# caprilovel/ECG_Denoise

Hardware: AMD Instinct MI355X
Metric: ECG windows/sec (512-sample, bs2048) train step; inference forward in infer_*_windows_per_s (higher is better)
Workload: dtype f32; 1 GPU; RA-LENet 'full' train step, 1-lead 512-sample windows, batch 2048/GPU (fwd+mse/SNR/RMSE+bwd+Adam), N(0,1) inputs seed 2023, random-init weights; global_batch=2048, batch_per_gpu=2048, parallelism=dp1, sync_bn=True

## Files before the change

ecg_denoise_amd/csrc/ral_bwd.hip:

```cpp
#ifdef RAL_STAMP_TU_BWD
#define RAL_STAMP_HERE
#endif
#include "ral_device.hpp"
#include "ral_kernels.hpp"
#include <stdio.h>
#include <stdlib.h>
#include <type_traits>

RAL_STAMPS_DEFINE(ral_debug_stamps)

RAL_DEV void lds_add4(double* red, int c, float4 v) {
  atomicAdd(red + c, (double)v.x); atomicAdd(red + c + 1, (double)v.y); atomicAdd(red + c + 2, (double)v.z); atomicAdd(red + c + 3, (double)v.w);
}

template <int C, int NCH>
__global__ __launch_bounds__(512) void k_mlp_bwd(const float* __restrict__ dx2, const float* __restrict__ x1,
                                                 const float* __restrict__ upre, BlockP w, BlockP wt, BlockP gr,
                                                 float* __restrict__ dupre, float* __restrict__ dx1,
                                                 float* __restrict__ do_hm, float* __restrict__ a2c0, int N, int B,
                                                 int NE ) {
  extern __shared__ float4 smem4[];
  constexpr int LD = LDof<C>::v, HC = 4 * C / NCH, LDU = LDof<HC>::v, LPR = C / 4;
  float* Ds = reinterpret_cast<float*>(smem4);
  float* Gs = Ds + N * LD;
  float* Us = Gs + N * LD;
  float* A0 = Us + N * LDU;
  float* DC0 = A0 + N + 2;
  float* U0 = DC0 + N + 2;
  float* C0 = U0 + N;
  float* red = C0 + N;
  const int RPP = blockDim.x / LPR;
  const int cq = (threadIdx.x % LPR) * 4;
  const bool le = w.le != nullptr;
  float lw0 = 0.f, lw1 = 0.f, lw2 = 0.f;
  if (le) { lw0 = w.le[0]; lw1 = w.le[1]; lw2 = w.le[2]; }
  const float4 gam2 = *reinterpret_cast<const float4*>(w.ln2w + cq);
  float gle0 = 0.f, gle1 = 0.f, gle2 = 0.f;
  float4 dgam = make_float4(0.f, 0.f, 0.f, 0.f), dbet = make_float4(0.f, 0.f, 0.f, 0.f);

  RAL_STAMP_INIT();
  for (int win = blockIdx.x; win < B; win += gridDim.x) {
    const size_t wo = (size_t)win * N * C;
    RAL_STAMP_AT(15);
    copy_in(Ds, LD, dx2 + wo, C, N, C);
#pragma unroll 1
    for (int ch = 0; ch < NCH; ++ch) {
      const int j0 = ch * HC;
      copy_in(Us, LDU, upre + (size_t)win * N * 4 * C + j0, 4 * C, N, HC);
      __syncthreads();
      RAL_STAMP_AT(0);
      if (le && ch == 0) {
        for (int i = threadIdx.x; i < N + 2; i += blockDim.x) {
          const bool halo = (i == 0 || i == N + 1);
          const float u = halo ? 0.f : Us[(i - 1) * LDU];
          A0[i] = (halo || i > NE) ? 0.f : gelu_f(u);
          DC0[i] = 0.f;
          if (!halo) U0[i - 1] = u;
// ... 899 lines not shown
  const f32x2 k01 = {kv.x, kv.y}, k23 = {kv.z, kv.w}, v01 = {vv.x, vv.y}, v23 = {vv.z, vv.w};
  f32x2 dk01 = {0.f, 0.f}, dk23 = {0.f, 0.f}, dv01 = {0.f, 0.f}, dv23 = {0.f, 0.f};
  for (int qt = 0; qt < N; qt += 4) {
    float4 qr[4], dr[4];
    float2 st[4];
#pragma unroll
    for (int j = 0; j < 4; ++j) { qr[j] = Q4[qt + j]; dr[j] = D4[qt + j]; st[j] = S2[qt + j]; }
#pragma unroll
    for (int j = 0; j < 4; ++j) {
      const f32x2 qa = {qr[j].x, qr[j].y}, qb2 = {qr[j].z, qr[j].w}, da = {dr[j].x, dr[j].y}, db = {dr[j].z, dr[j].w};
      f32x2 t = k01 * qa;
      t = pk_fma(k23, qb2, t);
      f32x2 u = v01 * da;
      u = pk_fma(v23, db, u);
      float hs = t[0] + t[1], hd = u[0] + u[1];
      asm volatile("" : "+v"(hs), "+v"(hd));
      f32x2 sd = {hs, hd};
      sd += f32x2{st[j].x, st[j].y};
      const float p = __builtin_amdgcn_exp2f(sd[0]);
      const float ds = p * sd[1];
      dk01 = pk_fma(splat2(ds), qa, dk01);
      dk23 = pk_fma(splat2(ds), qb2, dk23);
      dv01 = pk_fma(splat2(p), da, dv01);
      dv23 = pk_fma(splat2(p), db, dv23);
    }
  }
  if (kidx < N) {
    float4* dk = reinterpret_cast<float4*>(dqkv) + wbase + (size_t)(H + head) * N + kidx;
    float4* dv = reinterpret_cast<float4*>(dqkv) + wbase + (size_t)(2 * H + head) * N + kidx;
    *dk = make_float4(dk01[0], dk01[1], dk23[0], dk23[1]);
    *dv = make_float4(dv01[0], dv01[1], dv23[0], dv23[1]);
  }
}

template <int C>
#ifndef RAL_QKVB_MINB
#define RAL_QKVB_MINB 1
#endif
__global__ __launch_bounds__(512, RAL_QKVB_MINB) void k_qkv_bwd(const float* dqkv, const float* x,
                                                 const float* __restrict__ pe, const float* dx1,
                                                 const float* extra, BlockP w, BlockP wt, BlockP gr,
                                                 float* __restrict__ dx, int N, int B) {
  extern __shared__ float4 smem4[];
  constexpr int LD = LDof<C>::v, LPR = C / 4;
  float* DQ = reinterpret_cast<float*>(smem4);
  float* Dh = DQ + N * 3 * C;
  float* red = Dh + N * LD;
  const int RPP = blockDim.x / LPR;
  const int cq = (threadIdx.x % LPR) * 4;
  const float sqrtC = sqrtf((float)C);
  const float4 gam1 = *reinterpret_cast<const float4*>(w.ln1w + cq);
  float4 dgam = make_float4(0.f, 0.f, 0.f, 0.f), dbet = make_float4(0.f, 0.f, 0.f, 0.f);
  const int wave = threadIdx.x >> 6, nw = blockDim.x >> 6, lane = threadIdx.x & 63, r = lane & 15, g = lane >> 4;
  constexpr int NQ = 6, NR = 2;
  const int n4 = N * 3 * C / 4;
  const bool pfq = n4 <= NQ * (int)blockDim.x;
  const int rbase = threadIdx.x / LPR;
  const float* const ex = extra ? extra : dx1;
  auto row_off = [&](int win, int u) -> size_t {
    return (size_t)win * N * C + (size_t)min(rbase + u * RPP, N - 1) * C + cq;
  };
  auto ld4 = [&](const float* base, size_t o) -> float4 { return *reinterpret_cast<const float4*>(base + o); };
  auto ld_dq = [&](int win, int u) -> float4 {
    return reinterpret_cast<const float4*>(dqkv + (size_t)win * N * 3 * C)[min((int)threadIdx.x + u * (int)blockDim.x, n4 - 1)];
  };
  auto st_dq = [&](int u, float4 v) {
    const int i = threadIdx.x + u * blockDim.x;
    if (i < n4) reinterpret_cast<float4*>(DQ)[i] = v;
  };
  float4 pe4[NR];
#pragma unroll
  for (int u = 0; u < NR; ++u) pe4[u] = *reinterpret_cast<const float4*>(pe + min(rbase + u * RPP, N - 1) * C + cq);
  auto ln_row = [&](size_t wo, int row, float4 v, float4 p, float4 d1, float4 e) {
    v = f4add(f4scale(v, sqrtC), p);
    float4 d; float rstd;
    ln_stats<LPR>(v, d, rstd);
    const float4 xh = f4scale(d, rstd);
    const float4 dh = *reinterpret_cast<const float4*>(Dh + row * LD + cq);
    const float4 dyh = f4mul(dh, gam1);
    constexpr float invC = 1.0f / C;
    const float m1 = group_sum<LPR>(f4hsum(dyh)) * invC;
    const float m2 = group_sum<LPR>(f4dot(dyh, xh)) * invC;
    const float k = rstd * sqrtC;
    float4 out = make_float4(k * (dyh.x - m1 - xh.x * m2), k * (dyh.y - m1 - xh.y * m2),
                             k * (dyh.z - m1 - xh.z * m2), k * (dyh.w - m1 - xh.w * m2));
    out = f4add(out, d1);
    if (extra) out = f4add(out, e);
    *reinterpret_cast<float4*>(dx + wo + (size_t)row * C + cq) = out;
    dgam = f4add(dgam, f4mul(dh, xh));
    dbet = f4add(dbet, dh);
  };

  float4 rx[NR], rd[NR], re[NR];
#pragma unroll
  for (int u = 0; u < NR; ++u) rx[u] = rd[u] = re[u] = make_float4(0.f, 0.f, 0.f, 0.f);
  {
    const int win0 = blockIdx.x;
    if (win0 < B) {
#pragma unroll
      for (int u = 0; u < NR; ++u) {
        const size_t o = row_off(win0, u);
        rx[u] = ld4(x, o); rd[u] = ld4(dx1, o); re[u] = ld4(ex, o);
      }
      if (pfq) {
        float4 q[NQ];
#pragma unroll
        for (int u = 0; u < NQ; ++u) q[u] = ld_dq(win0, u);
#pragma unroll
        for (int u = 0; u < NQ; ++u) st_dq(u, q[u]);
      } else {
        copy_flat(DQ, dqkv + (size_t)win0 * N * 3 * C, n4);
      }
    }
    __syncthreads();
  }
  for (int win = blockIdx.x; win < B; win += gridDim.x) {
    const size_t wo = (size_t)win * N * C;
    {
      auto run = [&](auto ttb_tag) {
        constexpr int TT = decltype(ttb_tag)::value;
        constexpr int mt = (C + 15) >> 4;
        const int tg = (N >> 4) / TT;
        for (int u = wave; u < mt * tg; u += nw) {
          const int m = u % mt, tgi = u / mt;
          f32x4 acc[TT];
#pragma unroll
          for (int tt = 0; tt < TT; ++tt) acc[tt] = f32x4{0.f, 0.f, 0.f, 0.f};
          gemm_wx<C, TT, false, LAY_HM>(wt.wqkv, 3 * C, m * 16, C, DQ, N, tgi * TT * 16, acc);
          gemm_wx<2 * C, TT, false, LAY_HM>(wt.wqkv + C, 3 * C, m * 16, C, DQ + (C / 4) * N * 4, N, tgi * TT * 16, acc);
          const int row0 = m * 16 + 4 * g;
          if (row0 < C) {
#pragma unroll
            for (int tt = 0; tt < TT; ++tt)
              *reinterpret_cast<float4*>(Dh + ((tgi * TT + tt) * 16 + r) * LD + row0) = tofloat4(acc[tt]);
          }
        }
      };
      const int nt = N >> 4;
      if ((nt & 3) == 0) run(std::integral_constant<int, 4>{});
      else if ((nt & 1) == 0) run(std::integral_constant<int, 2>{});
      else run(std::integral_constant<int, 1>{});
    }
    __syncthreads();
    const int nxt = win + gridDim.x;
    const bool more = nxt < B;
    const int pw = more ? nxt : win;
    float4 q[NQ], nx[NR], nd[NR], ne[NR];
#pragma unroll
    for (int u = 0; u < NQ; ++u) q[u] = ld_dq(pw, u);
#pragma unroll
    for (int u = 0; u < NR; ++u) {
      const size_t o = row_off(pw, u);
      nx[u] = ld4(x, o); nd[u] = ld4(dx1, o); ne[u] = ld4(ex, o);
    }
    asm volatile("" ::: "memory");
    __builtin_amdgcn_sched_barrier(0);
#pragma unroll
    for (int u = 0; u < NR; ++u) {
      const int row = rbase + u * RPP;
      if (row < N) ln_row(wo, row, rx[u], pe4[u], rd[u], re[u]);
    }
    for (int row = rbase + NR * RPP; row < N; row += RPP) {
      const size_t o = wo + (size_t)row * C + cq;
      ln_row(wo, row, *reinterpret_cast<const float4*>(x + o), *reinterpret_cast<const float4*>(pe + row * C + cq),
             *reinterpret_cast<const float4*>(dx1 + o), *reinterpret_cast<const float4*>(ex + o));
    }
    if (more) {
      if (pfq) {
#pragma unroll
        for (int u = 0; u < NQ; ++u) st_dq(u, q[u]);
      } else {
        copy_flat(DQ, dqkv + (size_t)nxt * N * 3 * C, n4);
      }
    }
#pragma unroll
    for (int u = 0; u < NR; ++u) { rx[u] = nx[u]; rd[u] = nd[u]; re[u] = ne[u]; }
    __syncthreads();
  }
  double* redd = reinterpret_cast<double*>(smem4);
  for (int i = threadIdx.x; i < 2 * C; i += blockDim.x) redd[i] = 0.;
  __syncthreads();
  lds_add4(redd, cq, dgam);
  lds_add4(redd, C + cq, dbet);
  __syncthreads();
  if ((int)threadIdx.x < C) {
#ifndef RAL_NOVECATOMICS
    atomicAdd(gr.ln1w + threadIdx.x, (float)redd[threadIdx.x]);
    atomicAdd(gr.ln1b + threadIdx.x, (float)redd[C + threadIdx.x]);
#endif
  }
}

template <int C>
__global__ __launch_bounds__(512, RAL_QKVB_MINB) void k_qkv_bwd_h(const float* dqkv, const float* x,
                                                 const float* __restrict__ pe, const float* dx1,
                                                 const float* extra, BlockP w, BlockP wt, const float* __restrict__ ptbase,
                                                 const _Float16* __restrict__ wtt, BlockP gr,
                                                 float* __restrict__ dx, unsigned* __restrict__ gmax, int N, int B,
                                                 int NS ) {
  extern __shared__ float4 smem4[];
  constexpr int LD = LDof<C>::v, LPR = C / 4, LDQ = ldb_of(3 * C);
  typedef _Float16 f16x4 __attribute__((ext_vector_type(4)));
  const int NT = N / NS, t0 = ((int)blockIdx.x % NS) * NT, items = B * NS;
  _Float16* Qh = reinterpret_cast<_Float16*>(smem4);
  const int qplane = NT * LDQ;
  float* Dh = reinterpret_cast<float*>(Qh + 2 * qplane);
  float* red = Dh + NT * LD;
  unsigned* smQ = reinterpret_cast<unsigned*>(red + 2 * C);
  const int RPP = blockDim.x / LPR;
// ... 131 lines not shown
  for (int i = threadIdx.x; i < 2 * C; i += blockDim.x) redd[i] = 0.;
  __syncthreads();
  lds_add4(redd, cq, dgam);
  lds_add4(redd, C + cq, dbet);
  __syncthreads();
  if ((int)threadIdx.x < C) {
    atomicAdd(gr.ln1w + threadIdx.x, (float)redd[threadIdx.x]);
    atomicAdd(gr.ln1b + threadIdx.x, (float)redd[C + threadIdx.x]);
  }
  if (gmax) {
    __syncthreads();
    if (threadIdx.x == 0) smQ[0] = 0u;
    __syncthreads();
    const float mq = group_max<64>(tmxq);
    if ((threadIdx.x & 63) == 0) atomicMax(smQ, __float_as_uint(mq));
    __syncthreads();
    if (threadIdx.x == 0) atomicMax(gmax + 3, smQ[0]);
  }
}

template <int D, bool SEP>
__global__ __launch_bounds__(256) void k_resample_bwd(const float* dy, const float* x,
                                                      const float* __restrict__ wred, const float* __restrict__ lnw,
                                                      float* __restrict__ g_lnw, float* __restrict__ g_lnb,
                                                      float* __restrict__ dx, int T, int Tv, int B) {
  extern __shared__ float4 smem4[];
  constexpr int LD = LDof<D>::v, LPR = D / 4, RPP = 256 / LPR;
  float* Ys = reinterpret_cast<float*>(smem4);
  float* Dh = Ys + T * LD;
  float* red = Dh + T * LD;
  const int cq = (threadIdx.x % LPR) * 4;
  const float4 gam = *reinterpret_cast<const float4*>(lnw + cq);
  float4 dgam = make_float4(0.f, 0.f, 0.f, 0.f), dbet = make_float4(0.f, 0.f, 0.f, 0.f);
  auto src_of = [&](size_t wo, int row) -> size_t {
    return SEP ? wo + sep_src(row, T, Tv, D) : wo + (size_t)row * D;
  };
  auto ln_row = [&](int row, size_t src, float4 v) {
    float4 d; float rstd;
    ln_stats<LPR>(v, d, rstd);
    if (row < T) {
      const float4 xh = f4scale(d, rstd);
      const float4 dh = *reinterpret_cast<const float4*>(Dh + row * LD + cq);
      const float4 dyh = f4mul(dh, gam);
      constexpr float invD = 1.0f / D;
      const float m1 = group_sum<LPR>(f4hsum(dyh)) * invD;
      const float m2 = group_sum<LPR>(f4dot(dyh, xh)) * invD;
      *reinterpret_cast<float4*>(dx + src + cq) =
          make_float4(rstd * (dyh.x - m1 - xh.x * m2), rstd * (dyh.y - m1 - xh.y * m2),
                      rstd * (dyh.z - m1 - xh.z * m2), rstd * (dyh.w - m1 - xh.w * m2));
      dgam = f4add(dgam, f4mul(dh, xh));
      dbet = f4add(dbet, dh);
    }
  };
  if (T == 4 * RPP) {
    constexpr int q = D / 4;
    float4 dv[4], xv[4];
#define RAL_REQ_DY(win_) do { const float4* s4_ = reinterpret_cast<const float4*>(dy + (size_t)(win_) * T * D); \
      _Pragma("unroll") for (int k = 0; k < 4; ++k) dv[k] = s4_[threadIdx.x + k * 256]; } while (0)
    if ((int)blockIdx.x < B) RAL_REQ_DY(blockIdx.x);
    else { dv[0] = dv[1] = dv[2] = dv[3] = make_float4(0.f, 0.f, 0.f, 0.f); }
    for (int win = blockIdx.x; win < B; win += gridDim.x) {
      const size_t wo = (size_t)win * T * D;
#pragma unroll
      for (int k = 0; k < 4; ++k) {
        const int i = threadIdx.x + k * 256;
        *reinterpret_cast<float4*>(Ys + (i / q) * LD + (i % q) * 4) = dv[k];
      }
      __syncthreads();
      size_t src4[4];
#pragma unroll
      for (int u = 0; u < 4; ++u) {
        src4[u] = src_of(wo, threadIdx.x / LPR + u * RPP);
        xv[u] = *reinterpret_cast<const float4*>(x + src4[u] + cq);
      }
      asm volatile("" ::: "memory");
      __builtin_amdgcn_sched_barrier(0);
      gemm_phase<D, TTBof<D>::v, false, LAY_TOK>(wred , D, D, Ys, LD, T >> 4, [&](int row0, int tok, f32x4 a) {
        *reinterpret_cast<float4*>(Dh + tok * LD + row0) = tofloat4(a);
      });
      __syncthreads();
      const int nxt = win + gridDim.x;
      RAL_REQ_DY(nxt < B ? nxt : win);
      asm volatile("" ::: "memory");
      __builtin_amdgcn_sched_barrier(0);
#pragma unroll
      for (int u = 0; u < 4; ++u) ln_row(threadIdx.x / LPR + u * RPP, src4[u], xv[u]);
    }
#undef RAL_REQ_DY
    __syncthreads();
  } else {
  for (int win = blockIdx.x; win < B; win += gridDim.x) {
    const size_t wo = (size_t)win * T * D;
    copy_in(Ys, LD, dy + wo, D, T, D);
    __syncthreads();
    gemm_phase<D, TTBof<D>::v, false, LAY_TOK>(wred , D, D, Ys, LD, T >> 4, [&](int row0, int tok, f32x4 a) {
      *reinterpret_cast<float4*>(Dh + tok * LD + row0) = tofloat4(a);
    });
    __syncthreads();
    for (int row0 = threadIdx.x / LPR; row0 < T; row0 += 4 * RPP) {
      float4 v4[4]; size_t src4[4];
#pragma unroll
      for (int u = 0; u < 4; ++u) {
        src4[u] = src_of(wo, min(row0 + u * RPP, T - 1));
        v4[u] = *reinterpret_cast<const float4*>(x + src4[u] + cq);
      }
#pragma unroll
      for (int u = 0; u < 4; ++u) ln_row(row0 + u * RPP, src4[u], v4[u]);
// ... 280 lines not shown
    H4(32, 4) H4(64, 4) H4(128, 4) H8(32, 1) H8(64, 1)
    S(8, 1) S(8, 2) S(8, 4) S(16, 1) S(16, 2) S(32, 1) S(32, 2)
    F3(8) F3(16) F3(32) F3(64) F3(128)
    default: launch_mlp_bwd_w(p, dx2, x1, w, gr, dx1, do_hm, N, B, want_dw, s);
  }
#undef H
#undef H4
#undef H8
#undef S
#undef F
#undef F3
}

int launch_attn_bwd(const AttnPlan& p, const float* qkv, const float* o_hm, const float* do_hm, const float* lse, const float* table,
                    float* gtable, float* dqkv, float* scratch, size_t scratch_floats, int N, int H, int Len, int B, hipStream_t s,
                    int NE, AttnTabReduce* defer) {
  using K = AttnKernel;
  if (p.scratch_floats > (scratch ? scratch_floats : 0)) return -1;
  const int hg = p.hg, items = B * (H / hg);
  const int grid = p.threads == 512 ? cap(items, 4096) : cap(items, GRID_ATTNB);
#define TILE(kern) { RAL_SET_LDS((kern), p.lds); \
    kern<<<grid, p.threads, p.lds, s>>>(qkv, o_hm, do_hm, lse, table, gtable, dqkv, N, H, hg, Len, B); } return 0;
  int rows = 0;
  switch (p.kernel) {
    case K::BWD_RAG:
      RAL_SET_LDS((k_attn_bwd<1, 0, true, true>), p.lds);
      k_attn_bwd<1, 0, true, true><<<grid, p.threads, p.lds, s>>>(qkv, o_hm, do_hm, lse, table, gtable, dqkv, N, H, hg, Len, B, NE);
      return 0;
    case K::BWD_G1: TILE((k_attn_bwd<1>))
    case K::BWD_G2: TILE((k_attn_bwd<2>))
    case K::BWD_G2_N32: TILE((k_attn_bwd<2, 32, false>))
    case K::BWD_G2_N64_TAB: TILE((k_attn_bwd<2, 64, true>))
    case K::BWD_V: {
      const int ntask = B * H * ((N + 63) / 64), g = (ntask + 3) / 4;
      k_attn_bwd_vq<<<g, 256, 0, s>>>(qkv, o_hm, do_hm, lse, dqkv, scratch, N, H, ntask);
      k_attn_bwd_vkv<<<g, 256, 0, s>>>(qkv, do_hm, scratch, dqkv, N, H, ntask);
      return 0;
    }
    case K::BWD_MH4: case K::BWD_MH4_TAB: case K::BWD_MH8: case K::BWD_MH8_TAB:
      rows = launch_attn_bwd_mh(p, qkv, o_hm, do_hm, lse, table, dqkv, scratch, N, H, Len, B, s); break;
    case K::BWD_M32: case K::BWD_M32_TAB: case K::BWD_M64: case K::BWD_M64_TAB: case K::BWD_M128: case K::BWD_M128_TAB:
      rows = launch_attn_bwd_m(p, qkv, o_hm, do_hm, lse, table, dqkv, scratch, N, H, Len, B, s); break;
    default: rows = launch_attn_bwd_w(p, qkv, o_hm, do_hm, lse, table, dqkv, scratch, N, H, Len, B, s);
  }
#undef TILE
  if (p.table_partials) {
    const AttnTabReduce r{scratch, gtable, (2 * Len - 1) * H, rows};
    if (defer) *defer = r;
    else launch_attn_tpart_reduce(r, s);
  }
  return 0;
}

size_t qkv_bwd_lds(int C, int N) { return ((size_t)N * 3 * C + (size_t)N * ld_of(C) + 5 * C + 8) * sizeof(float); }
size_t qkv_bwd_h_lds(int C, int N) { return (size_t)2 * N * ldb_of(3 * C) * 2 + ((size_t)N * ld_of(C) + 2 * C + 2 * N) * 4; }
void launch_qkv_bwd(const BlockLaunch& p, const float* dqkv, const float* x, const float* pe, const float* dx1, const float* extra,
                    const BlockP& w, const BlockP& wt, const float* ptbase, const void* wtt, unsigned* gmax, const BlockP& gr, float* dx, int N, int B,
                    hipStream_t s) {
  using K = BlockKernel;
  const int grid = cap(B, GRID_QKVB);
  const _Float16* wp = reinterpret_cast<const _Float16*>(wtt);
#define H(c) case K::QKV_BWD_H_##c: RAL_SET_LDS((k_qkv_bwd_h<c>), p.lds); \
    k_qkv_bwd_h<c><<<grid, 512, p.lds, s>>>(dqkv, x, pe, dx1, extra, w, wt, ptbase, wp, gr, dx, gmax, N, B, 1); break;
#define F(c) case K::QKV_BWD_##c: RAL_SET_LDS((k_qkv_bwd<c>), p.lds); \
    k_qkv_bwd<c><<<grid, 512, p.lds, s>>>(dqkv, x, pe, dx1, extra, w, wt, gr, dx, N, B); break;
  switch (p.kernel) {
    H(32) H(64) H(128) F(8) F(16) F(32) F(64) F(128)
    default: block_launch_missing("launch_qkv_bwd", p);
  }
#undef H
#undef F
}

void launch_resample_bwd(int D, bool sep, const float* dy, const float* x, const float* wred, const float* lnw,
                         float* g_lnw, float* g_lnb, float* dx, int T, int Tv, int B, hipStream_t s) {
  const size_t lds = ((size_t)2 * T * ld_of(D) + 2 * D + 4) * sizeof(float);
  const int grid = cap(B, GRID_RESB);
#define CASE(d) case d: if (sep) { RAL_SET_LDS((k_resample_bwd<d, true>), lds); k_resample_bwd<d, true><<<grid, 256, lds, s>>>(dy, x, wred, lnw, g_lnw, g_lnb, dx, T, Tv, B); } \
                        else { RAL_SET_LDS((k_resample_bwd<d, false>), lds); k_resample_bwd<d, false><<<grid, 256, lds, s>>>(dy, x, wred, lnw, g_lnw, g_lnb, dx, T, Tv, B); } break;
  switch (D) { CASE(8) CASE(16) CASE(32) CASE(64) CASE(128) }
#undef CASE
}

void launch_final_bwd(int leads, const float* dy, const float* u0, const float* x0, const float* w, float* gw,
                      float* gb, float* dz, int L, int Lp, int B, hipStream_t s) {
  const int grid = ew_grid((size_t)B * Lp, 1024);
  if (leads == 1) k_final_bwd<1><<<grid, 256, 0, s>>>(dy, u0, x0, w, gw, gb, dz, L, Lp, B);
  else k_final_bwd<2><<<grid, 256, 0, s>>>(dy, u0, x0, w, gw, gb, dz, L, Lp, B);
}

void launch_bn8_bwd_stats(const float* dy, const float* a0, const float* ss, double* out, size_t ntok, hipStream_t s) {
  k_bn8_bwd_stats<<<ew_grid(ntok, 1024), 256, 0, s>>>(dy, a0, ss, out, ntok);
}

void launch_conv1_bwd(int leads, const float* dy, const float* a0, const float* x, const float* ss, const float* bnw,
                      const double* bst, double count, float* gw, float* gb, float* dz, int L, int Lp, int B, hipStream_t s,
                      float* gbnw, float* gbnb, double share) {
  const int grid = ew_grid((size_t)B * Lp, 1024);
  if (leads == 1) k_conv1_bwd<1><<<grid, 256, 0, s>>>(dy, a0, x, ss, bnw, bst, count, gw, gb, dz, L, Lp, B, gbnw, gbnb, share);
  else k_conv1_bwd<2><<<grid, 256, 0, s>>>(dy, a0, x, ss, bnw, bst, count, gw, gb, dz, L, Lp, B, gbnw, gbnb, share);
}

void launch_conv1_bwd_frozen(int leads, const float* dy, const float* a0, const float* x, const float* ss, const float* bnw,
                             float* gw, float* gb, float* dz, int L, int Lp, int B, hipStream_t s, float* gbnw, float* gbnb) {
  const int grid = ew_grid((size_t)B * Lp, 1024);
  if (leads == 1) k_conv1_bwd_frozen<1><<<grid, 256, 0, s>>>(dy, a0, x, ss, bnw, nullptr, 1.0, gw, gb, dz, L, Lp, B, gbnw, gbnb, 1.0);
  else k_conv1_bwd_frozen<2><<<grid, 256, 0, s>>>(dy, a0, x, ss, bnw, nullptr, 1.0, gw, gb, dz, L, Lp, B, gbnw, gbnb, 1.0);
}

void launch_conv1_bwd_dx(int leads, const float* dz, const float* w, float* dx, int L, int Lp, int B, hipStream_t s) {
  const int grid = ew_grid((size_t)B * L);
  if (leads == 1) k_conv1_bwd_dx<1><<<grid, 256, 0, s>>>(dz, w, dx, L, Lp, B);
  else k_conv1_bwd_dx<2><<<grid, 256, 0, s>>>(dz, w, dx, L, Lp, B);
}
```

ecg_denoise_amd/csrc/ral_fwd.hip:

```cpp
#ifdef RAL_STAMP_TU_FWD
#define RAL_STAMP_HERE
#endif
#include "ral_device.hpp"
#include "ral_kernels.hpp"
#include <stdio.h>
#include <stdlib.h>
#include <type_traits>

template <int C>
__global__ __launch_bounds__(256) void k_qkv_fwd(const float* __restrict__ x, const float* __restrict__ pe,
                                                 BlockP w, float* __restrict__ qkv, int N, int B) {
  extern __shared__ float4 smem4[];
  float* Hs = reinterpret_cast<float*>(smem4);
  constexpr int LD = LDof<C>::v, LPR = C / 4, RPP = 256 / LPR;
  const float sqrtC = sqrtf((float)C);
  const int cq = (threadIdx.x % LPR) * 4;
  const float4 gam = *reinterpret_cast<const float4*>(w.ln1w + cq);
  const float4 bet = *reinterpret_cast<const float4*>(w.ln1b + cq);
  for (int win = blockIdx.x; win < B; win += gridDim.x) {
    const float* xw = x + (size_t)win * N * C;
    for (int row = threadIdx.x / LPR; row < N; row += RPP) {
      float4 v = *reinterpret_cast<const float4*>(xw + row * C + cq);
      const float4 p = *reinterpret_cast<const float4*>(pe + row * C + cq);
      v = f4add(f4scale(v, sqrtC), p);
      float4 d; float rstd;
      ln_stats<LPR>(v, d, rstd);
      *reinterpret_cast<float4*>(Hs + row * LD + cq) = f4add(f4mul(f4scale(d, rstd), gam), bet);
    }
    __syncthreads();
    float* qw = qkv + (size_t)win * 3 * N * C;
    gemm_phase<C, TTBof<C>::v, false, LAY_TOK>(w.wqkv, C, 3 * C, Hs, LD, N >> 4, [&](int row0, int tok, f32x4 a) {
      float4 v = f4add(tofloat4(a), *reinterpret_cast<const float4*>(w.bqkv + row0));
      if (row0 < C) v = f4scale(v, 0.5f);
      *reinterpret_cast<float4*>(qw + ((size_t)(row0 >> 2) * N + tok) * 4) = v;
    });
    __syncthreads();
  }
}

template <int C, int GT>
__global__ __launch_bounds__(256) void k_qkv_fwd_h(const float* __restrict__ x, const float* __restrict__ pe,
                                                      BlockP w, const _Float16* __restrict__ wt,
                                                      float* __restrict__ qkv, int N, int B) {
  extern __shared__ float4 smem4[];
  _Float16* Hh = reinterpret_cast<_Float16*>(smem4);
  constexpr int LDB = ldb_of(C), LPR = C / 4, RPP = 256 / LPR, TT = 4;
  constexpr int MT = (3 * C / 16) % 8 == 0 ? 2 : 1;
  constexpr int xplane = GT * LDB;
  typedef _Float16 f16x4 __attribute__((ext_vector_type(4)));
  const float sqrtC = sqrtf((float)C);
  const int cq = (threadIdx.x % LPR) * 4;
  const float sg = asc_get(w.asc, ASC_LN1);
  const float4 gam = f4scale(*reinterpret_cast<const float4*>(w.ln1w + cq), sg);
  const float4 bet = f4scale(*reinterpret_cast<const float4*>(w.ln1b + cq), sg);
  const int wave = threadIdx.x >> 6, lane = threadIdx.x & 63, r = lane & 15, g = lane >> 4;
  const long total = (long)B * N;
  const int ngroups = (int)((total + GT - 1) / GT);
// ... 911 lines not shown
        const float4 v = *reinterpret_cast<const float4*>(Xs + row * LD + cq);
        float4 d; float rstd;
        ln_stats<LPR>(v, d, rstd);
        put_split(Gh, gplane, row * LDG + cq, f4add(f4mul(f4scale(d, rstd), gam), bet));
      }
    }
    __syncthreads();
    RAL_STAMP_AT(3);
    float* upw = upre_out ? upre_out + wo * 4 : nullptr;
    float* x2w = x2_out + wo;
    const float* addw = sum_out ? addend + wo : nullptr;
    float* sumw = sum_out ? sum_out + wo : nullptr;
#pragma unroll 1
    for (int ch = 0; ch < NCH; ++ch) {
      const int j0 = ch * HC;
      gemm_phase_h2<C, (NTH == 256 ? -1 : 0)>(w1h, C / 32, j0 / 16, 0, HC, w.b1 + j0, wun1, Gh, gplane, LDG, T >> 4, [&](int row0, int tok, f32x4 a) {
        const float4 u = tofloat4(a);
        if (upw) *reinterpret_cast<float4*>(upw + (size_t)tok * 4 * C + j0 + row0) = u;
        float4 h = make_float4(gelu_f(u.x), gelu_f(u.y), gelu_f(u.z), gelu_f(u.w));
        if (le) {
          if (ch == 0 && row0 == 0) A0[tok + 1 + 2 * (tok / N)] = h.x;
          h = make_float4(gelu_f(h.x), gelu_f(h.y), gelu_f(h.z), gelu_f(h.w));
        }
        put_split(Uh, uplane, tok * LDU + row0, f4scale(h, sh));
      });
      __syncthreads();
      RAL_STAMP_AT(4);
      if (le && ch == 0) {
        for (int n = threadIdx.x; n < T; n += NTH) {
          const int a = n + 1 + 2 * (n / N);
          const H2 s = f16_split2(gelu_f(lw0 * A0[a - 1] + lw1 * A0[a] + lw2 * A0[a + 1]) * sh);
          Uh[n * LDU] = s.a; Uh[uplane + n * LDU] = s.b;
        }
        __syncthreads();
      }
      RAL_STAMP_AT(5);
      gemm_phase_h2<HC>(w2h, 4 * C / 32, 0, j0 / 32, C, ch == 0 ? w.b2 : nullptr, wun2, Uh, uplane, LDU, T >> 4, [&](int row0, int tok, f32x4 a) {
        float4* px = reinterpret_cast<float4*>(Xs + tok * LD + row0);
        const float4 v = f4add(*px, tofloat4(a));
        if (ch == NCH - 1) {
          *reinterpret_cast<float4*>(x2w + (size_t)tok * C + row0) = v;
          if (sumw) *reinterpret_cast<float4*>(sumw + (size_t)tok * C + row0) = f4add(v, *reinterpret_cast<const float4*>(addw + (size_t)tok * C + row0));
        }
        else *px = v;
      });
      __syncthreads();
      RAL_STAMP_AT(6);
    }
  }
}


template <int D, bool SEP>
__global__ __launch_bounds__(256) void k_resample_fwd(const float* __restrict__ x, const float* __restrict__ wred,
                                                      const float* __restrict__ lnw, const float* __restrict__ lnb,
                                                      const float* __restrict__ skip, float* __restrict__ y,
                                                      int T, int Tv, int B) {
  extern __shared__ float4 smem4[];
  float* Hs = reinterpret_cast<float*>(smem4);
  constexpr int LD = LDof<D>::v, LPR = D / 4, RPP = 256 / LPR;
  const int cq = (threadIdx.x % LPR) * 4;
  const float4 gam = *reinterpret_cast<const float4*>(lnw + cq);
  const float4 bet = *reinterpret_cast<const float4*>(lnb + cq);
  for (int win = blockIdx.x; win < B; win += gridDim.x) {
    const float* xw = x + (size_t)win * T * D;
    for (int row = threadIdx.x / LPR; row < T; row += RPP) {
      const float* src = SEP ? xw + sep_src(row, T, Tv, D) : xw + (size_t)row * D;
      const float4 v = *reinterpret_cast<const float4*>(src + cq);
      float4 d; float rstd;
      ln_stats<LPR>(v, d, rstd);
      *reinterpret_cast<float4*>(Hs + row * LD + cq) = f4add(f4mul(f4scale(d, rstd), gam), bet);
    }
    __syncthreads();
    float* yw = y + (size_t)win * T * D;
    const float* sw = skip ? skip + (size_t)win * T * D : nullptr;
    gemm_phase<D, TTBof<D>::v, false, LAY_TOK>(wred, D, D, Hs, LD, T >> 4, [&](int row0, int tok, f32x4 a) {
      float4 v = tofloat4(a);
      if (sw) v = f4add(v, *reinterpret_cast<const float4*>(sw + (size_t)tok * D + row0));
      *reinterpret_cast<float4*>(yw + (size_t)tok * D + row0) = v;
    });
    __syncthreads();
  }
}

__global__ void k_add(const float* __restrict__ a, const float* __restrict__ b, float* __restrict__ y, size_t n4) {
  for (size_t i = (size_t)blockIdx.x * blockDim.x + threadIdx.x; i < n4; i += (size_t)gridDim.x * blockDim.x)
    reinterpret_cast<float4*>(y)[i] = f4add(reinterpret_cast<const float4*>(a)[i], reinterpret_cast<const float4*>(b)[i]);
}

static constexpr int GRID_FWD = 4096;
static inline int grid_for(int items) { return items < GRID_FWD ? items : GRID_FWD; }

size_t qkv_fwd_lds(int C, int N) { return (size_t)N * ld_of(C) * sizeof(float); }
size_t qkv_fwd_h_lds(int C, int bufs) { return (size_t)bufs * 2 * 64 * ldb_of(C) * 2; }

void launch_qkv_fwd(const BlockLaunch& p, const float* x, const float* pe, const BlockP& w, const void* wt, float* qkv, int N, int B, hipStream_t s) {
  using K = BlockKernel;
  const _Float16* wtp = reinterpret_cast<const _Float16*>(wt);
  const long ngroups = ((long)B * N + 63) / 64;
#define H(c) case K::QKV_FWD_H_##c: RAL_SET_LDS((k_qkv_fwd_h<c, 64>), p.lds); \
    k_qkv_fwd_h<c, 64><<<(int)(ngroups < 512 ? ngroups : 512), p.threads, p.lds, s>>>(x, pe, w, wtp, qkv, N, B); break;
#define WS(c, per_cu) case K::QKV_FWD_WS_##c: RAL_SET_LDS((k_qkv_fwd_ws<c, 64>), p.lds); \
    k_qkv_fwd_ws<c, 64><<<(int)(ngroups < 256 * per_cu ? ngroups : 256 * per_cu), p.threads, p.lds, s>>>(x, pe, w, wtp, qkv, N, B); break;
#define F(c) case K::QKV_FWD_##c: k_qkv_fwd<c><<<grid_for(B), p.threads, p.lds, s>>>(x, pe, w, qkv, N, B); break;
  switch (p.kernel) {
    WS(64, 2) WS(128, 1) H(32) H(64) F(8) F(16) F(32) F(64) F(128)
    default: block_launch_missing("launch_qkv_fwd", p);
  }
#undef H
#undef WS
#undef F
}

void launch_attn_fwd(const AttnPlan& p, const float* qkv, float* o_hm, float* lse, const float* table, int N, int H, int Len,
                     int B, hipStream_t s, int NE) {
  using K = AttnKernel;
  const int hg = p.hg, grid = grid_for(B * (H / hg));
#define TILE(kern) { RAL_SET_LDS((kern), p.lds); kern<<<grid, p.threads, p.lds, s>>>(qkv, o_hm, lse, table, N, H, hg, Len, B); } break;
  const int ntask = B * H * ((N + 63) / 64);
  switch (p.kernel) {
    case K::FWD_RAG:
      RAL_SET_LDS((k_attn_fwd<1, 0, true, false, true>), p.lds);
      k_attn_fwd<1, 0, true, false, true><<<grid, p.threads, p.lds, s>>>(qkv, o_hm, lse, table, N, H, hg, Len, B, NE);
      break;
    case K::FWD_G1: TILE((k_attn_fwd<1>))
    case K::FWD_G2: TILE((k_attn_fwd<2>))
    case K::FWD_G2_F16: TILE((k_attn_fwd<2, 0, true, true>))
    case K::FWD_G2_N32: TILE((k_attn_fwd<2, 32, false>))
    case K::FWD_T32: TILE((k_attn_fwd_t32<2, false>))
    case K::FWD_T32_TAB: TILE((k_attn_fwd_t32<2, true>))
    case K::FWD_V: k_attn_fwd_v<false><<<(ntask + 3) / 4, 256, 0, s>>>(qkv, o_hm, lse, table, N, H, 0, ntask); break;
    case K::FWD_V_TAB: k_attn_fwd_v<true><<<(ntask + 3) / 4, 256, 0, s>>>(qkv, o_hm, lse, table, N, H, Len, ntask); break;
    default: launch_attn_fwd_w(p, qkv, o_hm, lse, table, N, H, Len, B, s);
  }
#undef TILE
}

size_t mlp_fwd_lds(int C, int N, int nch) {
  return ((size_t)2 * N * ld_of(C) + (size_t)N * ld_of(4 * C / nch) + N + 2 + 2) * sizeof(float);
}

size_t mlp_fwd_h_lds(int C, int T, int nch) {
  return (size_t)T * ld_of(C) * 4 + (size_t)2 * T * ldb_of(C) * 2 + (size_t)2 * T * ldb_of(4 * C / nch) * 2 + (T / 16 * 2 + T + 4) * 4;
}

void launch_mlp_fwd(const BlockLaunch& p, const float* x, const float* o, const BlockP& w, const float* pbase, const void* wh,
                    float* x1, float* upre, float* x2, int N, int B, hipStream_t s, int NE, const float* addend, float* sum_out) {
  using K = BlockKernel;
  if (NE <= 0 || NE > N) NE = N;
  const _Float16* whp = reinterpret_cast<const _Float16*>(wh);
  const int grid = grid_for(B);
#define H(c, n, t) case K::MLP_FWD_H_##c##_##n: RAL_SET_LDS((k_mlp_fwd_h<c, n, t>), p.lds); \
    k_mlp_fwd_h<c, n, t><<<grid, t, p.lds, s>>>(x, o, w, pbase, whp, x1, upre, x2, N, B, 1, addend, sum_out); break;
#define F(c, n) case K::MLP_FWD_##c##_##n: RAL_SET_LDS((k_mlp_fwd<c, n>), p.lds); \
    k_mlp_fwd<c, n><<<grid, 512, p.lds, s>>>(x, o, w, x1, upre, x2, N, B, NE, addend, sum_out); break;
#define F3(c) F(c, 1) F(c, 2) F(c, 4)
  switch (p.kernel) {
    H(32, 1, 512) H(32, 2, 512) H(32, 4, 512)
    H(64, 1, 256) H(64, 8, 256) H(128, 4, 256) H(128, 8, 256)
    F3(8) F3(16) F3(32) F3(64) F3(128)
    default: launch_mlp_fwd_w(p, x, o, w, x1, x2, N, B, s);
  }
#undef H
#undef F
#undef F3
}

void launch_resample_fwd(int D, bool sep, const float* x, const float* wred, const float* lnw, const float* lnb,
                         const float* skip, float* y, int T, int Tv, int B, hipStream_t s) {
  const size_t lds = (size_t)T * ld_of(D) * sizeof(float);
#define CASE(d) case d: if (sep) k_resample_fwd<d, true><<<grid_for(B), 256, lds, s>>>(x, wred, lnw, lnb, skip, y, T, Tv, B); \
                        else k_resample_fwd<d, false><<<grid_for(B), 256, lds, s>>>(x, wred, lnw, lnb, skip, y, T, Tv, B); break;
  switch (D) { CASE(8) CASE(16) CASE(32) CASE(64) CASE(128) CASE(256) }
#undef CASE
}

void launch_add(const float* a, const float* b, float* y, size_t n, hipStream_t s) {
  const size_t n4 = n / 4;
  k_add<<<(int)((n4 + 255) / 256 < 8192 ? (n4 + 255) / 256 : 8192), 256, 0, s>>>(a, b, y, n4);
}
```

ecg_denoise_amd/csrc/ral_kernels.hpp:

```cpp
#pragma once
#include <hip/hip_runtime.h>
#include <stddef.h>
#include "ral_device.hpp"
#include "ral_attn_plan.hpp"
#include "ral_block_plan.hpp"

void launch_tile_planes(const float* params, void* wt, const void* desc, int ndesc, int nwork, int unscaled_residual, hipStream_t s);
void launch_act_scales(const float* params, const void* desc, float* asc, int nblk, hipStream_t s);
size_t qkv_fwd_lds(int C, int N);
size_t qkv_fwd_h_lds(int C, int bufs);
void launch_qkv_fwd(const BlockLaunch& p, const float* x, const float* pe, const BlockP& w, const void* wt , float* qkv, int N, int B, hipStream_t s);
size_t mlp_fwd_lds(int C, int N, int nch);
size_t mlp_fwd_h_lds(int C, int T, int nch);
size_t mlp_fwd_w_lds(int C, bool f16);
void launch_mlp_fwd(const BlockLaunch& p, const float* x, const float* o, const BlockP& w, const float* pbase, const void* wt,
                    float* x1, float* upre, float* x2, int N, int B, hipStream_t s, int NE = 0 ,
                    const float* addend = nullptr, float* sum_out = nullptr );
void launch_mlp_fwd_w(const BlockLaunch& p, const float* x, const float* o, const BlockP& w, float* x1, float* x2, int N, int B, hipStream_t s);
size_t mlp_bwd_w_lds(int C, bool h16, int* threads);
void launch_mlp_bwd_w(const BlockLaunch& p, const float* dx2, const float* x1, const BlockP& w, const BlockP& gr, float* dx1, float* do_hm, int N, int B,
                      bool want_dw, hipStream_t s);
void launch_resample_fwd(int D, bool sep, const float* x, const float* wred, const float* lnw, const float* lnb,
                         const float* skip, float* y, int T, int Tv , int B, hipStream_t s);
void launch_add(const float* a, const float* b, float* y, size_t n, hipStream_t s);

void launch_conv1_fwd(int leads, int mode, const float* x, const float* w, const float* b, float* out, double* stats,
                      const float* bnw, const float* bnb, const float* rmean, const float* rvar, int L, int Lp , int B,
                      hipStream_t s, float* out2 = nullptr, float* ss = nullptr);
void launch_bn_train8(const double* stats, double count, const float* bnw, const float* bnb, float* ss, float* rmean, float* rvar,
                      const float* a0, float* x0, size_t ntok, hipStream_t s);
void launch_final_fwd(int leads, const float* u0, const float* x0, const float* w, const float* b, float* y, int L, int Lp,
                      int B, hipStream_t s);
void launch_loss(const float* pred, const float* target, float* dy, float* snr, float* rmse, double* loss_sum,
                 int n, int B, float gscale, hipStream_t s, double* fin = nullptr, double fin_scale = 1.0, int fin3 = 0);
void launch_zero_bwd(float* grads, size_t nfloat, double* sums, int nsums, unsigned* gmax, int ngmax, hipStream_t s);
void launch_adam(float* p, const float* g, float* m, float* v, size_t n, double lr, double b1, double b2, double eps,
                 int step, float gscale, hipStream_t s, double* zero64 = nullptr );

void launch_transpose_mats(const float* src, float* dst, const void* desc, int nmat, int total, hipStream_t s);

size_t mlp_bwd_lds(int C, int N, int nch);
size_t mlp_bwd_s_lds(int C, int N);
size_t mlp_bwd_s_flush_lds(int C);
size_t mlp_bwd_h_lds(int C, int N, int nch, bool small);
void launch_mlp_bwd(const BlockLaunch& p, const float* dx2, const float* x1, const float* upre, const BlockP& w,
                    const BlockP& wt, const float* ptbase, const void* wtt, unsigned* gmax, const BlockP& gr, float* dupre, float* dx1, float* do_hm,
                    float* a2c0, int N, int B, bool want_dw, hipStream_t s, int NE = 0 );
void launch_attn_fwd(const AttnPlan& p, const float* qkv, float* o_hm, float* lse, const float* table, int N, int H, int Len,
                     int B, hipStream_t s, int NE = 0);
void launch_attn_fwd_w(const AttnPlan& p, const float* qkv, float* o_hm, float* lse, const float* table, int N, int H, int Len, int B, hipStream_t s);
struct AttnTabReduce { const float* tpart; float* gtable; int ntab, nrow; };
void launch_attn_tpart_reduce(const AttnTabReduce& r, hipStream_t s);
int launch_attn_bwd(const AttnPlan& p, const float* qkv, const float* o_hm, const float* do_hm, const float* lse, const float* table,
                    float* gtable, float* dqkv, float* scratch, size_t scratch_floats, int N, int H, int Len, int B, hipStream_t s,
                    int NE = 0, AttnTabReduce* defer = nullptr);
int launch_attn_bwd_w(const AttnPlan& p, const float* qkv, const float* o_hm, const float* do_hm, const float* lse, const float* table,
                      float* dqkv, float* tpart, int N, int H, int Len, int B, hipStream_t s);
int launch_attn_bwd_m(const AttnPlan& p, const float* qkv, const float* o_hm, const float* do_hm, const float* lse, const float* table,
                      float* dqkv, float* tpart, int N, int H, int Len, int B, hipStream_t s);
int launch_attn_bwd_mh(const AttnPlan& p, const float* qkv, const float* o_hm, const float* do_hm, const float* lse, const float* table,
                       float* dqkv, float* tpart, int N, int H, int Len, int B, hipStream_t s);
int attn_wave_grid(const void* kernel, size_t lds, int ntask, int occ_cap, int max_rows);
size_t qkv_bwd_lds(int C, int N);
size_t qkv_bwd_h_lds(int C, int N);
void launch_qkv_bwd(const BlockLaunch& p, const float* dqkv, const float* x, const float* pe, const float* dx1, const float* extra,
                    const BlockP& w, const BlockP& wt, const float* ptbase, const void* wtt , unsigned* gmax,
                    const BlockP& gr, float* dx, int N, int B, hipStream_t s);
void launch_resample_bwd(int D, bool sep, const float* dy, const float* x, const float* wred, const float* lnw,
                         float* g_lnw, float* g_lnb, float* dx, int T, int Tv, int B, hipStream_t s);
void launch_final_bwd(int leads, const float* dy, const float* u0, const float* x0, const float* w, float* gw,
                      float* gb, float* dz, int L, int Lp, int B, hipStream_t s);
void launch_bn8_bwd_stats(const float* dy, const float* a0, const float* ss, double* out, size_t ntok, hipStream_t s);
void launch_conv1_bwd(int leads, const float* dy, const float* a0, const float* x, const float* ss, const float* bnw,
                      const double* bst, double count, float* gw, float* gb, float* dz, int L, int Lp, int B, hipStream_t s,
                      float* gbnw, float* gbnb , double share);
void launch_conv1_bwd_frozen(int leads, const float* dy, const float* a0, const float* x, const float* ss, const float* bnw,
                             float* gw, float* gb, float* dz, int L, int Lp, int B, hipStream_t s, float* gbnw, float* gbnb);
void launch_conv1_bwd_dx(int leads, const float* dz, const float* w, float* dx, int L, int Lp, int B, hipStream_t s);

bool dw_chunk(int C, int prod , int N, bool split, int* tc, size_t* lds);
void launch_block_dw(const BlockPlan& p, const float* dx2, const float* upre, const float* a2c0, const float* dupre, const float* x1,
                     const float* dx1, const float* o_hm, const float* dqkv, const float* x, const float* pe,
                     const BlockP& w, const BlockP& gr, int N, int B, int ksplit, const unsigned* gmax, hipStream_t s);
void launch_resample_dw(int D, bool sep, const float* dy, const float* x, const float* lnw, const float* lnb,
                        float* dW, int T, int Tv, int B, int ksplit, hipStream_t s);
```

Measured before the change: 166,300 windows/s.

## Stage weights in LDS and prefetch next window in resample and qkv kernels

Adds fast paths to the resample forward and backward kernels for D<=64 with T*D==4096. They copy the reduction weight into LDS once per block and prefetch the next window's inputs into registers while the current window's GEMM runs. The forward grid is capped at 512 blocks so each block loops over several windows. The qkv backward kernel moves its next-window prefetch ahead of the GEMM, stages wqkv in LDS when C<=32, and replaces a __syncthreads with lds_barrier. It also adds C-API wrappers for these kernels. The cost is more LDS and register pressure, which may lower occupancy.

```diff
diff --git a/ecg_denoise_amd/csrc/ral_bwd.hip b/ecg_denoise_amd/csrc/ral_bwd.hip
--- a/ecg_denoise_amd/csrc/ral_bwd.hip
+++ b/ecg_denoise_amd/csrc/ral_bwd.hip
@@ -3,6 +3,8 @@
 #endif
 #include "ral_device.hpp"
 #include "ral_kernels.hpp"
+#include "ral_model.hpp"
+#include "../../include/ralenet.h"
 #include <stdio.h>
 #include <stdlib.h>
 #include <type_traits>
@@ -1008,6 +1010,10 @@
   const float4 gam1 = *reinterpret_cast<const float4*>(w.ln1w + cq);
   float4 dgam = make_float4(0.f, 0.f, 0.f, 0.f), dbet = make_float4(0.f, 0.f, 0.f, 0.f);
   const int wave = threadIdx.x >> 6, nw = blockDim.x >> 6, lane = threadIdx.x & 63, r = lane & 15, g = lane >> 4;
+  constexpr bool WLDS = C <= 32;
+  constexpr int LDWT = WLDS ? 3 * C + 4 : 3 * C;
+  float* Wl = Dh + N * LD + 5 * C + 8;
+  const float* const wq = WLDS ? Wl : wt.wqkv;
   constexpr int NQ = 6, NR = 2;
   const int n4 = N * 3 * C / 4;
   const bool pfq = n4 <= NQ * (int)blockDim.x;
@@ -1068,10 +1074,24 @@
         copy_flat(DQ, dqkv + (size_t)win0 * N * 3 * C, n4);
       }
     }
+    if constexpr (WLDS) copy_in(Wl, LDWT, wt.wqkv, 3 * C, C, 3 * C);
     __syncthreads();
   }
   for (int win = blockIdx.x; win < B; win += gridDim.x) {
     const size_t wo = (size_t)win * N * C;
+    const int nxt = win + gridDim.x;
+    const bool more = nxt < B;
+    const int pw = more ? nxt : win;
+    float4 q[NQ], nx[NR], nd[NR], ne[NR];
+#pragma unroll
+    for (int u = 0; u < NQ; ++u) q[u] = ld_dq(pw, u);
+#pragma unroll
+    for (int u = 0; u < NR; ++u) {
+      const size_t o = row_off(pw, u);
+      nx[u] = ld4(x, o); nd[u] = ld4(dx1, o); ne[u] = ld4(ex, o);
+    }
+    asm volatile("" ::: "memory");
+    __builtin_amdgcn_sched_barrier(0);
     {
       auto run = [&](auto ttb_tag) {
         constexpr int TT = decltype(ttb_tag)::value;
@@ -1082,8 +1102,8 @@
           f32x4 acc[TT];
 #pragma unroll
           for (int tt = 0; tt < TT; ++tt) acc[tt] = f32x4{0.f, 0.f, 0.f, 0.f};
-          gemm_wx<C, TT, false, LAY_HM>(wt.wqkv, 3 * C, m * 16, C, DQ, N, tgi * TT * 16, acc);
-          gemm_wx<2 * C, TT, false, LAY_HM>(wt.wqkv + C, 3 * C, m * 16, C, DQ + (C / 4) * N * 4, N, tgi * TT * 16, acc);
+          gemm_wx<C, TT, false, LAY_HM>(wq, LDWT, m * 16, C, DQ, N, tgi * TT * 16, acc);
+          gemm_wx<2 * C, TT, false, LAY_HM>(wq + C, LDWT, m * 16, C, DQ + (C / 4) * N * 4, N, tgi * TT * 16, acc);
           const int row0 = m * 16 + 4 * g;
           if (row0 < C) {
 #pragma unroll
@@ -1097,20 +1117,7 @@
       else if ((nt & 1) == 0) run(std::integral_constant<int, 2>{});
       else run(std::integral_constant<int, 1>{});
     }
-    __syncthreads();
-    const int nxt = win + gridDim.x;
-    const bool more = nxt < B;
-    const int pw = more ? nxt : win;
-    float4 q[NQ], nx[NR], nd[NR], ne[NR];
-#pragma unroll
-    for (int u = 0; u < NQ; ++u) q[u] = ld_dq(pw, u);
-#pragma unroll
-    for (int u = 0; u < NR; ++u) {
-      const size_t o = row_off(pw, u);
-      nx[u] = ld4(x, o); nd[u] = ld4(dx1, o); ne[u] = ld4(ex, o);
-    }
-    asm volatile("" ::: "memory");
-    __builtin_amdgcn_sched_barrier(0);
+    lds_barrier();
 #pragma unroll
     for (int u = 0; u < NR; ++u) {
       const int row = rbase + u * RPP;
@@ -1348,7 +1355,46 @@
       dbet = f4add(dbet, dh);
     }
   };
-  if (T == 4 * RPP) {
+  if (D <= 64 && T == 4 * RPP) {
+    constexpr int q = D / 4;
+    float* Ws = Dh + T * LD;
+    float4 dv[4], xv[4], ndv[4], nxv[4];
+    size_t src4[4], nsrc4[4];
+#define RAL_REQ_WIN(win_, dv_, xv_, src_) do { const size_t wo_ = (size_t)(win_) * T * D; \
+      const float4* s4_ = reinterpret_cast<const float4*>(dy + wo_); \
+      _Pragma("unroll") for (int k = 0; k < 4; ++k) { \
+        dv_[k] = s4_[threadIdx.x + k * 256]; \
+        src_[k] = src_of(wo_, threadIdx.x / LPR + k * RPP); \
+        xv_[k] = *reinterpret_cast<const float4*>(x + src_[k] + cq); } } while (0)
+    if ((int)blockIdx.x < B) RAL_REQ_WIN(blockIdx.x, dv, xv, src4);
+    else {
+#pragma unroll
+      for (int k = 0; k < 4; ++k) { dv[k] = xv[k] = make_float4(0.f, 0.f, 0.f, 0.f); src4[k] = 0; }
+    }
+    copy_in(Ws, LD, wred, D, D, D);
+    for (int win = blockIdx.x; win < B; win += gridDim.x) {
+#pragma unroll
+      for (int k = 0; k < 4; ++k) {
+        const int i = threadIdx.x + k * 256;
+        *reinterpret_cast<float4*>(Ys + (i / q) * LD + (i % q) * 4) = dv[k];
+      }
+      lds_barrier();
+      const int nxt = win + gridDim.x;
+      RAL_REQ_WIN(nxt < B ? nxt : win, ndv, nxv, nsrc4);
+      asm volatile("" ::: "memory");
+      __builtin_amdgcn_sched_barrier(0);
+      gemm_phase<D, TTBof<D>::v, false, LAY_TOK>(Ws , LD, D, Ys, LD, T >> 4, [&](int row0, int tok, f32x4 a) {
+        *reinterpret_cast<float4*>(Dh + tok * LD + row0) = tofloat4(a);
+      });
+      lds_barrier();
+#pragma unroll
+      for (int u = 0; u < 4; ++u) ln_row(threadIdx.x / LPR + u * RPP, src4[u], xv[u]);
+#pragma unroll
+      for (int k = 0; k < 4; ++k) { dv[k] = ndv[k]; xv[k] = nxv[k]; src4[k] = nsrc4[k]; }
+    }
+#undef RAL_REQ_WIN
+    __syncthreads();
+  } else if (T == 4 * RPP) {
     constexpr int q = D / 4;
     float4 dv[4], xv[4];
 #define RAL_REQ_DY(win_) do { const float4* s4_ = reinterpret_cast<const float4*>(dy + (size_t)(win_) * T * D); \
@@ -1735,7 +1781,9 @@
   return 0;
 }
 
-size_t qkv_bwd_lds(int C, int N) { return ((size_t)N * 3 * C + (size_t)N * ld_of(C) + 5 * C + 8) * sizeof(float); }
+size_t qkv_bwd_lds(int C, int N) {
+  return ((size_t)N * 3 * C + (size_t)N * ld_of(C) + 5 * C + 8 + (C <= 32 ? (size_t)C * (3 * C + 4) : 0)) * sizeof(float);
+}
 size_t qkv_bwd_h_lds(int C, int N) { return (size_t)2 * N * ldb_of(3 * C) * 2 + ((size_t)N * ld_of(C) + 2 * C + 2 * N) * 4; }
 void launch_qkv_bwd(const BlockLaunch& p, const float* dqkv, const float* x, const float* pe, const float* dx1, const float* extra,
                     const BlockP& w, const BlockP& wt, const float* ptbase, const void* wtt, unsigned* gmax, const BlockP& gr, float* dx, int N, int B,
@@ -1757,12 +1805,45 @@
 
 void launch_resample_bwd(int D, bool sep, const float* dy, const float* x, const float* wred, const float* lnw,
                          float* g_lnw, float* g_lnb, float* dx, int T, int Tv, int B, hipStream_t s) {
-  const size_t lds = ((size_t)2 * T * ld_of(D) + 2 * D + 4) * sizeof(float);
+  const size_t lds = ((size_t)(2 * T + (T * D == 4096 && D <= 64 ? D : 0)) * ld_of(D) + 2 * D + 4) * sizeof(float);
   const int grid = cap(B, GRID_RESB);
 #define CASE(d) case d: if (sep) { RAL_SET_LDS((k_resample_bwd<d, true>), lds); k_resample_bwd<d, true><<<grid, 256, lds, s>>>(dy, x, wred, lnw, g_lnw, g_lnb, dx, T, Tv, B); } \
                         else { RAL_SET_LDS((k_resample_bwd<d, false>), lds); k_resample_bwd<d, false><<<grid, 256, lds, s>>>(dy, x, wred, lnw, g_lnw, g_lnb, dx, T, Tv, B); } break;
   switch (D) { CASE(8) CASE(16) CASE(32) CASE(64) CASE(128) }
 #undef CASE
+}
+
+extern "C" int ral_resample_backward(const float* dy, const float* x, const float* wred_t, const float* lnw, float* g_lnw, float* g_lnb,
+                                     float* dx, int D, int separate, int T, int Tv, int B, ral_stream s) {
+  if (!dy || !x || !wred_t || !lnw || !g_lnw || !g_lnb || !dx) return ral_fail("resample_backward: null pointer");
+  if (resample_args("resample_backward", D, T, Tv, B)) return -1;
+  launch_resample_bwd(D, separate != 0, dy, x, wred_t, lnw, g_lnw, g_lnb, dx, T, Tv, B, (hipStream_t)s);
+  HIP_OK(hipGetLastError());
+  return 0;
+}
+
+extern "C" int ral_qkv_backward(const float* dqkv, const float* x, const float* pe, const float* dx1, const float* extra,
+                                const float* ln1w, const float* wqkv_t, float* g_ln1w, float* g_ln1b, float* dx, int C, int N, int B,
+                                ral_stream s) {
+  if (!dqkv || !x || !pe || !dx1 || !ln1w || !wqkv_t || !g_ln1w || !g_ln1b || !dx) return ral_fail("qkv_backward: null pointer");
+  if (C != 8 && C != 16 && C != 32 && C != 64 && C != 128) return ral_fail("qkv_backward: C must be 8, 16, 32, 64 or 128 (got %d)", C);
+  if (N < 16 || N % 16 != 0 || (size_t)N * C > 8192) return ral_fail("qkv_backward: N must be a multiple of 16 with N * C <= 8192 (N=%d C=%d)", N, C);
+  if (B < 1) return ral_fail("qkv_backward: B must be positive (got %d)", B);
+  using K = BlockKernel;
+  const K kern = C == 8 ? K::QKV_BWD_8 : C == 16 ? K::QKV_BWD_16 : C == 32 ? K::QKV_BWD_32 : C == 64 ? K::QKV_BWD_64 : K::QKV_BWD_128;
+  const BlockLaunch p{kern, "", 512, qkv_bwd_lds(C, N), 0, false};
+  BlockP w{}, wt{}, gr{};
+  w.ln1w = const_cast<float*>(ln1w);
+  wt.wqkv = const_cast<float*>(wqkv_t);
+  gr.ln1w = g_ln1w, gr.ln1b = g_ln1b;
+  launch_qkv_bwd(p, dqkv, x, pe, dx1, extra, w, wt, nullptr, nullptr, nullptr, gr, dx, N, B, (hipStream_t)s);
+  HIP_OK(hipGetLastError());
+  return 0;
+}
+
+extern "C" int ral_chain_grid_cap(int which) {
+  if (which < 0 || which > 2) return ral_fail("chain_grid_cap: which must be 0, 1 or 2 (got %d)", which);
+  return which == 0 ? resample_fwd_grid_cap() : which == 1 ? GRID_RESB : GRID_QKVB;
 }
 
 void launch_final_bwd(int leads, const float* dy, const float* u0, const float* x0, const float* w, float* gw,
diff --git a/ecg_denoise_amd/csrc/ral_fwd.hip b/ecg_denoise_amd/csrc/ral_fwd.hip
--- a/ecg_denoise_amd/csrc/ral_fwd.hip
+++ b/ecg_denoise_amd/csrc/ral_fwd.hip
@@ -3,6 +3,8 @@
 #endif
 #include "ral_device.hpp"
 #include "ral_kernels.hpp"
+#include "ral_model.hpp"
+#include "../../include/ralenet.h"
 #include <stdio.h>
 #include <stdlib.h>
 #include <type_traits>
@@ -1020,9 +1022,9 @@
 
 
 template <int D, bool SEP>
-__global__ __launch_bounds__(256) void k_resample_fwd(const float* __restrict__ x, const float* __restrict__ wred,
+__global__ __launch_bounds__(256) void k_resample_fwd(const float* x, const float* __restrict__ wred,
                                                       const float* __restrict__ lnw, const float* __restrict__ lnb,
-                                                      const float* __restrict__ skip, float* __restrict__ y,
+                                                      const float* skip, float* __restrict__ y,
                                                       int T, int Tv, int B) {
   extern __shared__ float4 smem4[];
   float* Hs = reinterpret_cast<float*>(smem4);
@@ -1030,6 +1032,51 @@
   const int cq = (threadIdx.x % LPR) * 4;
   const float4 gam = *reinterpret_cast<const float4*>(lnw + cq);
   const float4 bet = *reinterpret_cast<const float4*>(lnb + cq);
+  if (D <= 64 && T == 4 * RPP) {
+    constexpr int q = D / 4;
+    float* Ss = Hs + T * LD;
+    float* Ws = Ss + T * LD;
+    const float* const sb = skip ? skip : lnw;
+    const int smask = skip ? -1 : 0;
+    float4 xv[4], sv[4];
+#define RAL_REQ_WIN(win_) do { const size_t wo_ = (size_t)(win_) * T * D; \
+      const float4* s4_ = reinterpret_cast<const float4*>(sb + (skip ? wo_ : (size_t)0)); \
+      _Pragma("unroll") for (int u = 0; u < 4; ++u) { \
+        const int row_ = threadIdx.x / LPR + u * RPP; \
+        xv[u] = *reinterpret_cast<const float4*>(x + wo_ + (SEP ? sep_src(row_, T, Tv, D) : (size_t)row_ * D) + cq); \
+        sv[u] = s4_[(threadIdx.x + u * 256) & smask]; } } while (0)
+    if ((int)blockIdx.x < B) RAL_REQ_WIN(blockIdx.x);
+    else {
+#pragma unroll
+      for (int u = 0; u < 4; ++u) xv[u] = sv[u] = make_float4(0.f, 0.f, 0.f, 0.f);
+    }
+    copy_in(Ws, LD, wred, D, D, D);
+    for (int win = blockIdx.x; win < B; win += gridDim.x) {
+#pragma unroll
+      for (int u = 0; u < 4; ++u) {
+        const int row = threadIdx.x / LPR + u * RPP;
+        float4 d; float rstd;
+        ln_stats<LPR>(xv[u], d, rstd);
+        *reinterpret_cast<float4*>(Hs + row * LD + cq) = f4add(f4mul(f4scale(d, rstd), gam), bet);
+        const int i = threadIdx.x + u * 256;
+        *reinterpret_cast<float4*>(Ss + (i / q) * LD + (i % q) * 4) = sv[u];
+      }
+      lds_barrier();
+      const int nxt = win + gridDim.x;
+      RAL_REQ_WIN(nxt < B ? nxt : win);
+      asm volatile("" ::: "memory");
+      __builtin_amdgcn_sched_barrier(0);
+      float* yw = y + (size_t)win * T * D;
+      gemm_phase<D, TTBof<D>::v, false, LAY_TOK>(Ws, LD, D, Hs, LD, T >> 4, [&](int row0, int tok, f32x4 a) {
+        float4 v = tofloat4(a);
+        if (skip) v = f4add(v, *reinterpret_cast<const float4*>(Ss + tok * LD + row0));
+        *reinterpret_cast<float4*>(yw + (size_t)tok * D + row0) = v;
+      });
+      lds_barrier();
+    }
+#undef RAL_REQ_WIN
+    return;
+  }
   for (int win = blockIdx.x; win < B; win += gridDim.x) {
     const float* xw = x + (size_t)win * T * D;
     for (int row = threadIdx.x / LPR; row < T; row += RPP) {
@@ -1058,6 +1105,8 @@
 
 static constexpr int GRID_FWD = 4096;
 static inline int grid_for(int items) { return items < GRID_FWD ? items : GRID_FWD; }
+static constexpr int GRID_RESF = 512;
+int resample_fwd_grid_cap() { return GRID_RESF; }
 
 size_t qkv_fwd_lds(int C, int N) { return (size_t)N * ld_of(C) * sizeof(float); }
 size_t qkv_fwd_h_lds(int C, int bufs) { return (size_t)bufs * 2 * 64 * ldb_of(C) * 2; }
@@ -1136,11 +1185,30 @@
 
 void launch_resample_fwd(int D, bool sep, const float* x, const float* wred, const float* lnw, const float* lnb,
                          const float* skip, float* y, int T, int Tv, int B, hipStream_t s) {
-  const size_t lds = (size_t)T * ld_of(D) * sizeof(float);
-#define CASE(d) case d: if (sep) k_resample_fwd<d, true><<<grid_for(B), 256, lds, s>>>(x, wred, lnw, lnb, skip, y, T, Tv, B); \
-                        else k_resample_fwd<d, false><<<grid_for(B), 256, lds, s>>>(x, wred, lnw, lnb, skip, y, T, Tv, B); break;
+  const bool fast = T * D == 4096 && D <= 64;
+  const size_t lds = (size_t)(fast ? 2 * T + D : T) * ld_of(D) * sizeof(float);
+  const int grid = fast ? (B < GRID_RESF ? B : GRID_RESF) : grid_for(B);
+#define CASE(d) case d: if (sep) { RAL_SET_LDS((k_resample_fwd<d, true>), lds); k_resample_fwd<d, true><<<grid, 256, lds, s>>>(x, wred, lnw, lnb, skip, y, T, Tv, B); } \
+                        else { RAL_SET_LDS((k_resample_fwd<d, false>), lds); k_resample_fwd<d, false><<<grid, 256, lds, s>>>(x, wred, lnw, lnb, skip, y, T, Tv, B); } break;
   switch (D) { CASE(8) CASE(16) CASE(32) CASE(64) CASE(128) CASE(256) }
 #undef CASE
+}
+
+int resample_args(const char* who, int D, int T, int Tv, int B) {
+  if (D != 8 && D != 16 && D != 32 && D != 64 && D != 128) return ral_fail("%s: D must be 8, 16, 32, 64 or 128 (got %d)", who, D);
+  if (T < 16 || T % 16 != 0 || (size_t)T * D > 16384) return ral_fail("%s: T must be a multiple of 16 with T * D <= 16384 (T=%d D=%d)", who, T, D);
+  if (Tv < 2 || Tv > T || (Tv & 1)) return ral_fail("%s: Tv must be even in [2, T] (Tv=%d T=%d)", who, Tv, T);
+  if (B < 1) return ral_fail("%s: B must be positive (got %d)", who, B);
+  return 0;
+}
+
+extern "C" int ral_resample_forward(const float* x, const float* wred, const float* lnw, const float* lnb, const float* skip, float* y,
+                                    int D, int separate, int T, int Tv, int B, ral_stream s) {
+  if (!x || !wred || !lnw || !lnb || !y) return ral_fail("resample_forward: null pointer");
+  if (resample_args("resample_forward", D, T, Tv, B)) return -1;
+  launch_resample_fwd(D, separate != 0, x, wred, lnw, lnb, skip, y, T, Tv, B, (hipStream_t)s);
+  HIP_OK(hipGetLastError());
+  return 0;
 }
 
 void launch_add(const float* a, const float* b, float* y, size_t n, hipStream_t s) {
diff --git a/ecg_denoise_amd/csrc/ral_kernels.hpp b/ecg_denoise_amd/csrc/ral_kernels.hpp
--- a/ecg_denoise_amd/csrc/ral_kernels.hpp
+++ b/ecg_denoise_amd/csrc/ral_kernels.hpp
@@ -66,6 +66,8 @@
 void launch_qkv_bwd(const BlockLaunch& p, const float* dqkv, const float* x, const float* pe, const float* dx1, const float* extra,
                     const BlockP& w, const BlockP& wt, const float* ptbase, const void* wtt , unsigned* gmax,
                     const BlockP& gr, float* dx, int N, int B, hipStream_t s);
+int resample_fwd_grid_cap();
+int resample_args(const char* who, int D, int T, int Tv, int B);
 void launch_resample_bwd(int D, bool sep, const float* dy, const float* x, const float* wred, const float* lnw,
                          float* g_lnw, float* g_lnb, float* dx, int T, int Tv, int B, hipStream_t s);
 void launch_final_bwd(int leads, const float* dy, const float* u0, const float* x0, const float* w, float* gw,
```

New measurement: 166,200 windows/s (median of 2 runs). Within noise of the previous version (-0.1%).
